# dmar-bonn/ipp-marl

Measured on AMD Instinct MI355X. Metric: agent-env steps/s (4 UAVs, 256x256 grid, random policy, env-step HIP kernels), higher is better.
Workload: dtype f32

## Files before the change

ipp-marl_amd/csrc/terrain.hip:

```cpp
#include "ippm_internal.h"

#define IPPM_DOMAIN_TERRAIN 3u

static inline hipStream_t S_(void* s) { return reinterpret_cast<hipStream_t>(s); }

__global__ __launch_bounds__(256) void k_terrain_noise(const ippm_config* __restrict__ c, const int64_t* __restrict__ episode,
                                                       float* __restrict__ noise, size_t cells) {
  const int e = blockIdx.y;
  const uint64_t ep = (uint64_t)episode[e];
  const uint32_t k0 = (uint32_t)c->philox_seed, k1 = (uint32_t)(c->philox_seed >> 32);
  const uint32_t sw = ippm_stream_word(0u, 0u, IPPM_DOMAIN_TERRAIN);
  float* out = noise + (size_t)e * cells;
  const size_t groups = (cells + 3) >> 2;
  for (size_t g = (size_t)blockIdx.x * blockDim.x + threadIdx.x; g < groups; g += (size_t)gridDim.x * blockDim.x) {
    Philox4 ph = ippm_philox((uint32_t)g, (uint32_t)ep, sw, (uint32_t)(ep >> 32), k0, k1);
    float z[4];
#pragma unroll
    for (int h = 0; h < 2; ++h) {
      const float u1 = ((float)(ph.v[2 * h] >> 8) + 1.0f) * (1.0f / 16777216.0f);
      const float u2 = (float)(ph.v[2 * h + 1] >> 8) * (1.0f / 16777216.0f);
      const float r = sqrtf(-2.0f * logf(u1));
      float s, co;
      sincospif(2.0f * u2, &s, &co);
      z[2 * h] = r * co;
      z[2 * h + 1] = r * s;
    }
    const size_t base = g << 2;
    if (base + 3 < cells && (cells & 3) == 0) {
      *reinterpret_cast<float4*>(out + base) = make_float4(z[0], z[1], z[2], z[3]);
    } else {
      for (int q = 0; q < 4 && base + q < cells; ++q) out[base + q] = z[q];
    }
  }
}


__device__ __forceinline__ float2 cmul(float2 a, float2 b) {
#pragma clang fp contract(off)
  const float p = a.y * b.y, q = a.y * b.x;
  return make_float2(__builtin_fmaf(a.x, b.x, -p), __builtin_fmaf(a.x, b.y, q));
}
__device__ __forceinline__ uint32_t bitrev(uint32_t v, int bits) { return __brev(v) >> (32 - bits); }

__device__ __forceinline__ uint32_t terrain_call(int gx, int gy, int cx, int ky) {
  return (uint32_t)(cx & (gx / 2 - 1)) * (uint32_t)(gy / 2 + 1) + (uint32_t)ky;
}
__device__ __forceinline__ float2 terrain_bin_from(uint32_t w1, uint32_t w2, bool self, bool conj, float amp) {
  const float u1 = ((float)(w1 >> 8) + 1.0f) * (1.0f / 16777216.0f);
  const float u2 = (float)(w2 >> 8) * (1.0f / 16777216.0f);
  const float r = __builtin_sqrtf(-1.3862943611f * __builtin_amdgcn_logf(u1));
  const float sn = __builtin_amdgcn_sinf(u2), cs = __builtin_amdgcn_cosf(u2);
  if (self) return make_float2(amp * 1.41421356237f * r * cs, 0.0f);
  return make_float2(amp * r * cs, conj ? -amp * r * sn : amp * r * sn);
}
__device__ __forceinline__ float2 terrain_bin(uint64_t ep, uint32_t k0, uint32_t k1, int gx, int gy, int kx, int ky, float amp) {
  const bool edge = ky == 0 || 2 * ky == gy;
  int cx = kx;
  bool conj = false;
  if (edge && 2 * kx > gx) { cx = gx - kx; conj = true; }
  const bool self = edge && (cx == 0 || 2 * cx == gx);
  Philox4 ph = ippm_philox(terrain_call(gx, gy, cx, ky), (uint32_t)ep, ippm_stream_word(0u, 1u, IPPM_DOMAIN_TERRAIN), (uint32_t)(ep >> 32), k0, k1);
  const bool upper = 2 * cx >= gx;
  return terrain_bin_from(upper ? ph.v[2] : ph.v[0], upper ? ph.v[3] : ph.v[1], self, conj, amp);
}
__device__ __forceinline__ void terrain_bin_pair(uint64_t ep, uint32_t k0, uint32_t k1, int gx, int gy, int kx, int ky, float amp_lo,
                                                 float amp_hi, float2& lo, float2& hi) {
  Philox4 ph = ippm_philox(terrain_call(gx, gy, kx, ky), (uint32_t)ep, ippm_stream_word(0u, 1u, IPPM_DOMAIN_TERRAIN), (uint32_t)(ep >> 32), k0, k1);
  lo = terrain_bin_from(ph.v[0], ph.v[1], false, false, amp_lo);
  hi = terrain_bin_from(ph.v[2], ph.v[3], false, false, amp_hi);
}

__global__ __launch_bounds__(256) void k_terrain_spectrum(const ippm_config* __restrict__ c, const int64_t* __restrict__ episode,
                                                          const float* __restrict__ amp, float2* __restrict__ spec) {
  const int e = blockIdx.y, gx = c->grid_x, gy = c->grid_y, hy = gy / 2 + 1;
  const uint64_t ep = (uint64_t)episode[e];
  const uint32_t k0 = (uint32_t)c->philox_seed, k1 = (uint32_t)(c->philox_seed >> 32);
  for (int i = blockIdx.x * blockDim.x + threadIdx.x; i < gx * hy; i += gridDim.x * blockDim.x)
    spec[(size_t)e * gx * hy + i] = terrain_bin(ep, k0, k1, gx, gy, i / hy, i % hy, amp[i]);
}

__device__ constexpr float TWC[16] = {1.000000000f, 0.980785280f, 0.923879533f, 0.831469612f, 0.707106781f, 0.555570233f,
                                      0.382683432f, 0.195090322f, 0.000000000f, -0.195090322f, -0.382683432f, -0.555570233f,
                                      -0.707106781f, -0.831469612f, -0.923879533f, -0.980785280f};
__device__ constexpr float TWS[16] = {0.000000000f, 0.195090322f, 0.382683432f, 0.555570233f, 0.707106781f, 0.831469612f,
                                      0.923879533f, 0.980785280f, 1.000000000f, 0.980785280f, 0.923879533f, 0.831469612f,
                                      0.707106781f, 0.555570233f, 0.382683432f, 0.195090322f};

template <int R>
__device__ __forceinline__ void fft_reg(float2 (&a)[R]) {
  constexpr int LOG = R == 8 ? 3 : (R == 16 ? 4 : 5);
  static_assert((1 << LOG) == R, "fft_reg: R must be 8, 16 or 32");
#pragma unroll
  for (int i = 0; i < R; ++i) {
    int j = 0;
#pragma unroll
    for (int b = 0; b < LOG; ++b) j |= ((i >> b) & 1) << (LOG - 1 - b);
    if (i < j) {
      const float2 t = a[i];
      a[i] = a[j];
      a[j] = t;
    }
  }
#pragma unroll
  for (int s = 0; s < LOG; ++s) {
#pragma unroll
    for (int j = 0; j < R / 2; ++j) {
      const int half = 1 << s, pos = j & (half - 1), i0 = ((j >> s) << (s + 1)) + pos, i1 = i0 + half, t = pos * (16 >> s);
      const float2 u = a[i0], v = cmul(a[i1], make_float2(TWC[t], TWS[t]));
      a[i0] = make_float2(u.x + v.x, u.y + v.y);
      a[i1] = make_float2(u.x - v.x, u.y - v.y);
    }
  }
}

template <int N1, int N2, int Q>
struct FourStep {
  static constexpr int SEQ = N1 * (N2 + 1) + 1;
  static constexpr int THREADS = Q * (N1 > N2 ? N1 : N2);
  float2 xbuf[Q * SEQ];
  float2 twn[N1 * N2];

  __device__ __forceinline__ void init_twiddles(const float2* __restrict__ roots1024) {
    for (int i = threadIdx.x; i < N1 * N2; i += THREADS) twn[i] = roots1024[i * (1024 / (N1 * N2))];
    __syncthreads();
  }
  __device__ __forceinline__ void run(float2 (&v)[N1], float2 (&o)[N2], int q_in, int i2, bool in_active, int q_out, int k1,
                                      bool out_active) {
    if (in_active) {
      fft_reg<N1>(v);
#pragma unroll
      for (int k = 0; k < N1; ++k) xbuf[q_in * SEQ + k * (N2 + 1) + i2] = cmul(v[k], twn[i2 * k]);
    }
    __syncthreads();
    if (out_active) {
#pragma unroll
      for (int i = 0; i < N2; ++i) o[i] = xbuf[q_out * SEQ + k1 * (N2 + 1) + i];
      fft_reg<N2>(o);
    }
  }
};

__device__ __forceinline__ uint32_t order_key(float f) {
  const uint32_t b = __float_as_uint(f);
  return (b & 0x80000000u) ? ~b : (b | 0x80000000u);
}
__device__ __forceinline__ float key_value(uint32_t k) { return __uint_as_float((k & 0x80000000u) ? (k & 0x7FFFFFFFu) : ~k); }

template <int N1, int N2, int Q, bool GEN>
__global__ __launch_bounds__((FourStep<N1, N2, Q>::THREADS)) void k_terrain_fft_x(const ippm_config* __restrict__ c,
                                                                               const int64_t* __restrict__ episode,
                                                                               const float* __restrict__ amp,
                                                                               const float2* __restrict__ spec,
                                                                               float2* __restrict__ work,
                                                                               uint32_t* __restrict__ range_keys,
                                                                               const float2* __restrict__ roots1024, int key_stride) {
  __shared__ FourStep<N1, N2, Q> fs;
  const int e = blockIdx.y, gx = N1 * N2, gy = c->grid_y, hy = gy / 2 + 1, tid = threadIdx.x;
  const bool edge_wg = blockIdx.x == gridDim.x - 1;
  if (range_keys && blockIdx.x == 0 && tid == 0) {
    range_keys[key_stride * e] = 0xFFFFFFFFu;
    range_keys[key_stride * e + 1] = 0u;
    if (key_stride == 4) {
      range_keys[4 * e + 2] = 0u;
      range_keys[4 * e + 3] = 0u;
      if (e == 0) range_keys[4 * gridDim.y] = 0u;
    }
  }
  fs.init_twiddles(roots1024);
  const int q_in = tid % Q, i2 = tid / Q, k1 = tid % N1, q_out = tid / N1;
  const bool in_active = i2 < N2, out_active = q_out < Q;
  auto column = [&](int q) { return edge_wg ? (q == 0 ? 0 : (q == 1 ? gy / 2 : -1)) : (1 + (int)blockIdx.x * Q + q < gy / 2 ? 1 + (int)blockIdx.x * Q + q : -1); };
  float2 v[N1], o[N2];
  if (in_active) {
    const int ky = column(q_in);
    const uint64_t ep = GEN ? (uint64_t)episode[e] : 0;
    const uint32_t k0 = (uint32_t)c->philox_seed, k1s = (uint32_t)(c->philox_seed >> 32);
#pragma unroll
    for (int i1 = 0; i1 < N1; ++i1) v[i1] = make_float2(0.0f, 0.0f);
    if (ky >= 0) {
      if (GEN && edge_wg) {
#pragma unroll
        for (int i1 = 0; i1 < N1; ++i1) {
          const int kx = i1 * N2 + i2;
          v[i1] = terrain_bin(ep, k0, k1s, gx, gy, kx, ky, amp[(size_t)kx * hy + ky]);
        }
      } else if (GEN) {
#pragma unroll
        for (int i1 = 0; i1 < N1 / 2; ++i1) {
          const int kx = i1 * N2 + i2;
          terrain_bin_pair(ep, k0, k1s, gx, gy, kx, ky, amp[(size_t)kx * hy + ky], amp[(size_t)(kx + gx / 2) * hy + ky], v[i1], v[i1 + N1 / 2]);
        }
      } else {
#pragma unroll
        for (int i1 = 0; i1 < N1; ++i1) v[i1] = spec[((size_t)e * gx + i1 * N2 + i2) * hy + ky];
      }
    }
  }
  fs.run(v, o, q_in, i2, in_active, q_out, k1, out_active);
  const int ky_out = out_active ? column(q_out) : -1;
  if (ky_out >= 0) {
    float2* dst = work + ((size_t)e * hy + ky_out) * gx + k1;
#pragma unroll
    for (int k2 = 0; k2 < N2; ++k2) dst[N1 * k2] = o[k2];
  }
}

template <int N1, int N2, int Q, int MODE>
__global__ __launch_bounds__((FourStep<N1, N2, Q>::THREADS)) void k_terrain_fft_y(const ippm_config* __restrict__ c,
                                                                               const float2* __restrict__ work,
                                                                               float* __restrict__ field,
                                                                               uint32_t* __restrict__ range_keys,
                                                                               const float2* __restrict__ roots1024,
                                                                               uint32_t* __restrict__ truth32, int truth_words, int key_stride) {
  __shared__ FourStep<N1, N2, Q> fs;
  const int tid = threadIdx.x, gx = c->grid_x, gy = N1 * N2, hy = gy / 2 + 1;
  int e = blockIdx.y, part = blockIdx.x;
  __shared__ uint32_t s_ticket, s_keys[2];
  if (MODE == 3) {
    if (tid == 0) s_ticket = atomicAdd(range_keys + 4 * gridDim.y, 1u);
  }
  fs.init_twiddles(roots1024);
  if (MODE == 3) {
    const uint32_t tk = s_ticket;
    e = (int)(tk / gridDim.x);
    part = (int)(tk - (uint32_t)e * gridDim.x);
  }
  const int x0 = part * 2 * Q;
  const int q_in = tid % Q, i2 = tid / Q, k1 = tid % N1, q_out = tid / N1;
  const bool in_active = i2 < N2, out_active = q_out < Q;
  float2 v[N1], o[N2];
  if (in_active) {
    const float2* src = work + (size_t)e * hy * gx + x0 + 2 * q_in;
#pragma unroll
    for (int i1 = 0; i1 < N1; ++i1) {
      const int i = i1 * N2 + i2, m = 2 * i > gy ? gy - i : i;
      const float4 ab = *reinterpret_cast<const float4*>(src + (size_t)m * gx);
      float2 a = make_float2(ab.x, ab.y), b = make_float2(ab.z, ab.w);
      if (2 * i > gy) { a.y = -a.y; b.y = -b.y; }
      if (i == 0 || 2 * i == gy) { a.y = 0.0f; b.y = 0.0f; }
      v[i1] = make_float2(a.x - b.y, a.y + b.x);
    }
  }
  fs.run(v, o, q_in, i2, in_active, q_out, k1, out_active);
  if (MODE != 2) {
    float lo = INFINITY, hi = -INFINITY;
    if (out_active) {
      float* dst = field + ((size_t)e * gx + x0 + 2 * q_out) * gy + k1;
#pragma unroll
      for (int k2 = 0; k2 < N2; ++k2) {
        if (MODE == 0) {
          dst[N1 * k2] = o[k2].x;
          dst[(size_t)gy + N1 * k2] = o[k2].y;
        }
        lo = fminf(lo, fminf(o[k2].x, o[k2].y));
        hi = fmaxf(hi, fmaxf(o[k2].x, o[k2].y));
      }
    }
    if (range_keys) {
#pragma unroll
      for (int m = 32; m > 0; m >>= 1) {
        lo = fminf(lo, __shfl_xor(lo, m, 64));
        hi = fmaxf(hi, __shfl_xor(hi, m, 64));
      }
      __shared__ float s_lo[8], s_hi[8];
      constexpr int NW = FourStep<N1, N2, Q>::THREADS / 64;
      if ((tid & 63) == 0) { s_lo[tid >> 6] = lo; s_hi[tid >> 6] = hi; }
      __syncthreads();
      if (tid == 0) {
        for (int w = 1; w < NW; ++w) { lo = fminf(lo, s_lo[w]); hi = fmaxf(hi, s_hi[w]); }
        if (MODE != 3) {
          atomicMin(range_keys + key_stride * e, order_key(lo));
          atomicMax(range_keys + key_stride * e + 1, order_key(hi));
        } else {
          uint32_t* rec = range_keys + 4 * e;
          const uint32_t o1 = __hip_atomic_fetch_min(rec, order_key(lo), __ATOMIC_RELAXED, __HIP_MEMORY_SCOPE_AGENT);
          const uint32_t o2 = __hip_atomic_fetch_max(rec + 1, order_key(hi), __ATOMIC_RELAXED, __HIP_MEMORY_SCOPE_AGENT);
          asm volatile("s_waitcnt vmcnt(0)" : : "v"(o1), "v"(o2) : "memory");
          __hip_atomic_fetch_add(rec + 2, 1u, __ATOMIC_RELAXED, __HIP_MEMORY_SCOPE_AGENT);
          unsigned spins = 0;
          while (atomicCAS(rec + 2, 0xFFFFFFFFu, 0xFFFFFFFEu) < gridDim.x) {
            __builtin_amdgcn_s_sleep(64);
            if (++spins > (1u << 21)) {
              atomicExch(rec + 3, 0xDEAD0000u | (unsigned)part);
              break;
            }
          }
          s_keys[0] = atomicCAS(rec, 0xFFFFFFFFu, 0xFFFFFFFEu);
          s_keys[1] = atomicCAS(rec + 1, 0xFFFFFFFFu, 0xFFFFFFFEu);
        }
      }
    }
    if (MODE != 3) return;
    __syncthreads();
  }
  {
    static_assert(N1 == 8 || N1 == 16 || N1 == 32, "a chunk must not straddle a 32-bit word");
    const uint32_t key_lo = MODE == 3 ? s_keys[0] : range_keys[key_stride * e];
    const uint32_t key_hi = MODE == 3 ? s_keys[1] : range_keys[key_stride * e + 1];
    const float lo = key_value(key_lo), span = key_value(key_hi) - lo;
    const int lane = tid & 63, rows_per_wave = 64 / N1;
    const int my_q = (tid >> 6) * rows_per_wave + lane;
    const bool storer = lane < rows_per_wave && my_q < Q;
    uint32_t* out = truth32 + (size_t)e * truth_words;
    const size_t row_a = ((size_t)(x0 + 2 * my_q) * gy) >> 5, row_b = ((size_t)(x0 + 2 * my_q + 1) * gy) >> 5;
    uint32_t wa = 0, wb = 0;
#pragma unroll
    for (int k2 = 0; k2 < N2; ++k2) {
      const uint64_t ba = __ballot(out_active && (o[k2].x - lo) / span >= 0.5f);
      const uint64_t bb = __ballot(out_active && (o[k2].y - lo) / span >= 0.5f);
      const uint32_t mask = N1 == 32 ? 0xFFFFFFFFu : ((1u << (N1 & 31)) - 1u);
      const int sh = (k2 * N1) & 31;
      wa |= ((uint32_t)(ba >> ((N1 * lane) & 63)) & mask) << sh;
      wb |= ((uint32_t)(bb >> ((N1 * lane) & 63)) & mask) << sh;
      if (((k2 + 1) * N1) % 32 == 0) {
        if (storer) { out[row_a + ((k2 * N1) >> 5)] = wa; out[row_b + ((k2 * N1) >> 5)] = wb; }
        wa = 0; wb = 0;
      }
    }
  }
}

#define IPPM_PACK_PARTS 4
__global__ __launch_bounds__(1024) void k_terrain_pack(const float* __restrict__ field, uint8_t* __restrict__ truth, size_t cells,
                                                       size_t truth_bytes) {
  __shared__ float s_lo[16], s_hi[16];
  const int e = blockIdx.y, tid = threadIdx.x, lane = tid & 63, wave = tid >> 6, nwave = blockDim.x >> 6;
  const float* f = field + (size_t)e * cells;
  float lo = INFINITY, hi = -INFINITY;
  if ((cells & 3) == 0) {
    const float4* f4 = reinterpret_cast<const float4*>(f);
    const size_t n4 = cells >> 2;
#pragma unroll 4
    for (size_t i = tid; i < n4; i += blockDim.x) {
      const float4 v = f4[i];
      lo = fminf(fminf(lo, fminf(v.x, v.y)), fminf(v.z, v.w));
      hi = fmaxf(fmaxf(hi, fmaxf(v.x, v.y)), fmaxf(v.z, v.w));
    }
  } else {
    for (size_t i = tid; i < cells; i += blockDim.x) {
      const float v = f[i];
      lo = fminf(lo, v);
      hi = fmaxf(hi, v);
    }
  }
#pragma unroll
  for (int o = 32; o > 0; o >>= 1) {
    lo = fminf(lo, __shfl_xor(lo, o, 64));
    hi = fmaxf(hi, __shfl_xor(hi, o, 64));
  }
  if (lane == 0) { s_lo[wave] = lo; s_hi[wave] = hi; }
  __syncthreads();
  lo = s_lo[0];
  hi = s_hi[0];
  for (int w = 1; w < nwave; ++w) {
    lo = fminf(lo, s_lo[w]);
    hi = fmaxf(hi, s_hi[w]);
  }
  const float span = hi - lo;
  uint32_t* out = reinterpret_cast<uint32_t*>(truth + (size_t)e * truth_bytes);
  const size_t words = truth_bytes >> 2;
  const size_t chunks = (cells + 63) >> 6;
  for (size_t ch = (size_t)blockIdx.x * nwave + wave; ch < chunks; ch += (size_t)gridDim.x * nwave) {
    const size_t i = (ch << 6) + lane;
    const bool one = i < cells && (f[i] - lo) / span >= 0.5f;
    const uint64_t bits = __ballot(one);
    if (lane < 2 && 2 * ch + lane < words) out[2 * ch + lane] = (uint32_t)(bits >> (32 * lane));
  }
}

__global__ __launch_bounds__(256) void k_terrain_pack_keys(const float* __restrict__ field, const uint32_t* __restrict__ range_keys,
                                                           uint8_t* __restrict__ truth, size_t cells, size_t truth_bytes) {
  const int e = blockIdx.y, lane = threadIdx.x & 63, wave = threadIdx.x >> 6, nwave = blockDim.x >> 6;
  const float* f = field + (size_t)e * cells;
  const float lo = key_value(range_keys[2 * e]), span = key_value(range_keys[2 * e + 1]) - lo;
  uint32_t* out = reinterpret_cast<uint32_t*>(truth + (size_t)e * truth_bytes);
  const size_t words = truth_bytes >> 2, chunks = (cells + 63) >> 6;
  const size_t stride = (size_t)gridDim.x * nwave;
  for (size_t ch0 = (size_t)blockIdx.x * nwave + wave; ch0 < chunks; ch0 += 4 * stride) {
    float v[4];
#pragma unroll
    for (int u = 0; u < 4; ++u) {
      const size_t i = ((ch0 + u * stride) << 6) + lane;
      v[u] = i < cells ? f[i] : lo;
    }
#pragma unroll
    for (int u = 0; u < 4; ++u) {
      const size_t ch = ch0 + u * stride;
      const uint64_t bits = __ballot(((ch << 6) + lane) < cells && (v[u] - lo) / span >= 0.5f);
      if (ch < chunks && lane < 2 && 2 * ch + lane < words) out[2 * ch + lane] = (uint32_t)(bits >> (32 * lane));
    }
  }
}

typedef float terrain_f4 __attribute__((ext_vector_type(4)));
__global__ __launch_bounds__(256) void k_terrain_pack_keys4(const float* __restrict__ field, const uint32_t* __restrict__ range_keys,
                                                            uint8_t* __restrict__ truth, size_t cells, size_t truth_bytes) {
  const int e = blockIdx.y;
  const size_t g = (size_t)blockIdx.x * 256 + threadIdx.x;
  const float lo = key_value(range_keys[2 * e]), span = key_value(range_keys[2 * e + 1]) - lo;
  uint32_t nib = 0;
  if (4 * g < cells) {
    const terrain_f4 v = __builtin_nontemporal_load(reinterpret_cast<const terrain_f4*>(field + (size_t)e * cells) + g);
    nib = ((v.x - lo) / span >= 0.5f ? 1u : 0u) | ((v.y - lo) / span >= 0.5f ? 2u : 0u) | ((v.z - lo) / span >= 0.5f ? 4u : 0u) |
          ((v.w - lo) / span >= 0.5f ? 8u : 0u);
  }
  uint32_t w = nib << (4 * (threadIdx.x & 7));
  w |= __shfl_xor(w, 1, 64);
  w |= __shfl_xor(w, 2, 64);
  w |= __shfl_xor(w, 4, 64);
  const size_t word = g >> 3;
  if ((threadIdx.x & 7) == 0 && word < (truth_bytes >> 2)) reinterpret_cast<uint32_t*>(truth + (size_t)e * truth_bytes)[word] = w;
}

extern "C" int ippm_terrain_noise(ippm_ctx* ctx, const int64_t* episode, float* noise, int32_t n_envs, void* stream) {
  if (!ctx || !episode || !noise) { ippm_set_error("ippm_terrain_noise: null argument"); return -1; }
  if (n_envs <= 0) return 0;
  const size_t cells = (size_t)ctx->cfg.grid_x * ctx->cfg.grid_y;
  const int gx = (int)std::min<size_t>(64, (cells / 4 + 255) / 256);
  hipLaunchKernelGGL(k_terrain_noise, dim3(gx > 0 ? gx : 1, n_envs), dim3(256), 0, S_(stream), ctx->dcfg, episode, noise, cells);
  IPPM_LAUNCH_CHECK("terrain_noise");
  return 0;
}

extern "C" int ippm_terrain_pack(ippm_ctx* ctx, const float* field, const uint32_t* range_keys, uint8_t* truth, int32_t n_envs,
                                 void* stream) {
  if (!ctx || !field || !truth) { ippm_set_error("ippm_terrain_pack: null argument"); return -1; }
  if (n_envs <= 0) return 0;
  const size_t cells = (size_t)ctx->cfg.grid_x * ctx->cfg.grid_y;
  if (range_keys && cells % 4 == 0 && (reinterpret_cast<uintptr_t>(field) & 15) == 0) {
    IPPM_LAUNCH(ctx, IPPM_T_TERRAIN, k_terrain_pack_keys4, dim3((unsigned)((cells / 4 + 255) / 256), n_envs), dim3(256), S_(stream), field,
                       range_keys, truth, cells, ippm_truth_bytes(ctx->cfg.grid_x, ctx->cfg.grid_y));
    IPPM_LAUNCH_CHECK("terrain_pack_keys4");
    return 0;
  }
  if (range_keys) {
    const int gxb = (int)std::min<size_t>(64, ((cells + 63) / 64 + 15) / 16);
    hipLaunchKernelGGL(k_terrain_pack_keys, dim3(gxb > 0 ? gxb : 1, n_envs), dim3(256), 0, S_(stream), field, range_keys, truth, cells,
                       ippm_truth_bytes(ctx->cfg.grid_x, ctx->cfg.grid_y));
    IPPM_LAUNCH_CHECK("terrain_pack_keys");
    return 0;
  }
  hipLaunchKernelGGL(k_terrain_pack, dim3(IPPM_PACK_PARTS, n_envs), dim3(1024), 0, S_(stream), field, truth, cells,
                     ippm_truth_bytes(ctx->cfg.grid_x, ctx->cfg.grid_y));
  IPPM_LAUNCH_CHECK("terrain_pack");
  return 0;
}

static bool terrain_side_ok(int n) { return n == 128 || n == 256 || n == 512 || n == 1024; }

static int terrain_pow2_check(const ippm_ctx* ctx, const char* who) {
  if (!terrain_side_ok(ctx->cfg.grid_x) || !terrain_side_ok(ctx->cfg.grid_y)) {
    ippm_set_error(std::string(who) + ": grid sides must be 128, 256, 512 or 1024 (use ippm_terrain_noise + an FFT library otherwise)");
    return -1;
  }
  return 0;
}

#define TERRAIN_DISPATCH(n, CALL)                \
  switch (n) {                                   \
    case 128: { CALL(8, 16, 16); break; }        \
    case 256: { CALL(16, 16, 16); break; }       \
    case 512: { CALL(16, 32, 8); break; }        \
    default: { CALL(32, 32, 4); break; }         \
  }

extern "C" int ippm_terrain_spectrum(ippm_ctx* ctx, const int64_t* episode, const float* amp, float* spec, int32_t n_envs,
                                     void* stream) {
  if (!ctx || !episode || !amp || !spec) { ippm_set_error("ippm_terrain_spectrum: null argument"); return -1; }
  if (terrain_pow2_check(ctx, "ippm_terrain_spectrum")) return -1;
  if (n_envs <= 0) return 0;
  const int bins = ctx->cfg.grid_x * (ctx->cfg.grid_y / 2 + 1);
  hipLaunchKernelGGL(k_terrain_spectrum, dim3(std::min(64, (bins + 255) / 256), n_envs), dim3(256), 0, S_(stream), ctx->dcfg,
                     episode, amp, reinterpret_cast<float2*>(spec));
  IPPM_LAUNCH_CHECK("terrain_spectrum");
  return 0;
}

static int terrain_launch_x(ippm_ctx* ctx, const int64_t* episode, const float* amp, const float2* spec2, float2* work2,
                            uint32_t* range_keys, int n_envs, hipStream_t st, int key_stride = 2) {
  const int gx = ctx->cfg.grid_x, gy = ctx->cfg.grid_y;
#define LAUNCH_X(N1, N2, Q)                                                                                                  \
  {                                                                                                                          \
    const dim3 grid((gy / 2 - 1 + Q - 1) / Q + 1, n_envs), block(FourStep<N1, N2, Q>::THREADS);                              \
    if (spec2) IPPM_LAUNCH(ctx, IPPM_T_TERRAIN, (k_terrain_fft_x<N1, N2, Q, false>), grid, block, st, ctx->dcfg, episode, amp, spec2, work2, \
                           range_keys, ctx->d_roots, key_stride);                                                            \
    else IPPM_LAUNCH(ctx, IPPM_T_TERRAIN, (k_terrain_fft_x<N1, N2, Q, true>), grid, block, st, ctx->dcfg, episode, amp, spec2, work2,        \
                     range_keys, ctx->d_roots, key_stride);                                                                  \
  }
  TERRAIN_DISPATCH(gx, LAUNCH_X)
#undef LAUNCH_X
  IPPM_LAUNCH_CHECK("terrain_fft_x");
  return 0;
}

template <int MODE>
static int terrain_launch_y(ippm_ctx* ctx, const float2* work2, float* field, uint32_t* range_keys, uint8_t* truth, int n_envs,
                            hipStream_t st, int key_stride = 2) {
  const int gx = ctx->cfg.grid_x, gy = ctx->cfg.grid_y;
#define LAUNCH_Y(N1, N2, Q)                                                                                                  \
  IPPM_LAUNCH(ctx, IPPM_T_TERRAIN, (k_terrain_fft_y<N1, N2, Q, MODE>), dim3(gx / (2 * Q), n_envs), dim3(FourStep<N1, N2, Q>::THREADS), st, \
              ctx->dcfg, work2, field, range_keys, ctx->d_roots, reinterpret_cast<uint32_t*>(truth), (int)(ippm_truth_bytes(gx, gy) >> 2),       \
              MODE == 3 ? 4 : key_stride)
  TERRAIN_DISPATCH(gy, LAUNCH_Y)
#undef LAUNCH_Y
  IPPM_LAUNCH_CHECK("terrain_fft_y");
  return 0;
}

extern "C" int ippm_terrain_field(ippm_ctx* ctx, const int64_t* episode, const float* amp, const float* spec, float* work,
                                  float* field, uint32_t* range_keys, int32_t n_envs, void* stream) {
  if (!ctx || !work || !field) { ippm_set_error("ippm_terrain_field: null argument"); return -1; }
  if (!spec && (!episode || !amp)) { ippm_set_error("ippm_terrain_field: needs either spec or (episode, amp)"); return -1; }
  if (terrain_pow2_check(ctx, "ippm_terrain_field")) return -1;
  if (n_envs <= 0) return 0;
  if (int rc = terrain_launch_x(ctx, episode, amp, reinterpret_cast<const float2*>(spec), reinterpret_cast<float2*>(work), range_keys, n_envs,
                                S_(stream))) return rc;
  return terrain_launch_y<0>(ctx, reinterpret_cast<const float2*>(work), field, range_keys, nullptr, n_envs, S_(stream));
}

extern "C" int ippm_terrain_truth(ippm_ctx* ctx, const int64_t* episode, const float* amp, float* work, uint32_t* range_keys,
                                  uint8_t* truth, int32_t n_envs, void* stream) {
  if (!ctx || !episode || !amp || !work || !range_keys || !truth) { ippm_set_error("ippm_terrain_truth: null argument"); return -1; }
  if (terrain_pow2_check(ctx, "ippm_terrain_truth")) return -1;
  if (n_envs <= 0) return 0;
  if (int rc = terrain_launch_x(ctx, episode, amp, nullptr, reinterpret_cast<float2*>(work), range_keys, n_envs, S_(stream), 4)) return rc;
  if (ctx->knob_terrain_one_launch && ctx->cfg.grid_x <= 512)
    return terrain_launch_y<3>(ctx, reinterpret_cast<const float2*>(work), nullptr, range_keys, truth, n_envs, S_(stream), 4);
  if (int rc = terrain_launch_y<1>(ctx, reinterpret_cast<const float2*>(work), nullptr, range_keys, nullptr, n_envs, S_(stream), 4)) return rc;
  return terrain_launch_y<2>(ctx, reinterpret_cast<const float2*>(work), nullptr, range_keys, truth, n_envs, S_(stream), 4);
}
```

Baseline: 29.32 million.

## Fuse terrain 2D FFT and threshold pack into one per-env on-chip kernel

Adds a single-block-per-environment kernel that runs the x-direction FFT, transposes through shared memory, runs the y-direction FFT, reduces min/max in-block, and writes the packed truth bits. For square grids up to 256 it is used when the one-launch knob is off, replacing the global work buffer round trip, the atomic range keys and the separate launches. In exchange each environment runs in one workgroup with large register arrays, so parallelism is limited to n_envs blocks and register pressure may spill. Shared helpers are factored out of the existing kernels.

```diff
diff --git a/ipp-marl_amd/csrc/terrain.hip b/ipp-marl_amd/csrc/terrain.hip
--- a/ipp-marl_amd/csrc/terrain.hip
+++ b/ipp-marl_amd/csrc/terrain.hip
@@ -145,6 +145,65 @@
   return (b & 0x80000000u) ? ~b : (b | 0x80000000u);
 }
 __device__ __forceinline__ float key_value(uint32_t k) { return __uint_as_float((k & 0x80000000u) ? (k & 0x7FFFFFFFu) : ~k); }
+
+
+template <int N1, int N2>
+__device__ __forceinline__ void terrain_draw_column(float2 (&v)[N1], uint64_t ep, uint32_t k0, uint32_t k1s, const float* __restrict__ amp,
+                                                    int gy, int i2, int ky, bool edge) {
+  constexpr int gx = N1 * N2;
+  const int hy = gy / 2 + 1;
+  if (edge) {
+#pragma unroll
+    for (int i1 = 0; i1 < N1; ++i1) {
+      const int kx = i1 * N2 + i2;
+      v[i1] = terrain_bin(ep, k0, k1s, gx, gy, kx, ky, amp[(size_t)kx * hy + ky]);
+    }
+  } else {
+#pragma unroll
+    for (int i1 = 0; i1 < N1 / 2; ++i1) {
+      const int kx = i1 * N2 + i2;
+      terrain_bin_pair(ep, k0, k1s, gx, gy, kx, ky, amp[(size_t)kx * hy + ky], amp[(size_t)(kx + gx / 2) * hy + ky], v[i1], v[i1 + N1 / 2]);
+    }
+  }
+}
+
+template <int N1, int N2>
+__device__ __forceinline__ void terrain_row_pair(float2 (&v)[N1], const float2* src, size_t stride, int i2) {
+  constexpr int gy = N1 * N2;
+#pragma unroll
+  for (int i1 = 0; i1 < N1; ++i1) {
+    const int i = i1 * N2 + i2, m = 2 * i > gy ? gy - i : i;
+    const float4 ab = *reinterpret_cast<const float4*>(src + (size_t)m * stride);
+    float2 a = make_float2(ab.x, ab.y), b = make_float2(ab.z, ab.w);
+    if (2 * i > gy) { a.y = -a.y; b.y = -b.y; }
+    if (i == 0 || 2 * i == gy) { a.y = 0.0f; b.y = 0.0f; }
+    v[i1] = make_float2(a.x - b.y, a.y + b.x);
+  }
+}
+
+template <int N1, int N2, int Q>
+__device__ __forceinline__ void terrain_threshold_pack(const float2 (&o)[N2], bool out_active, int t, float lo, float span,
+                                                       uint32_t* __restrict__ out, int x0, int gy) {
+  static_assert(N1 == 8 || N1 == 16 || N1 == 32, "a chunk must not straddle a 32-bit word");
+  const int lane = t & 63, rows_per_wave = 64 / N1;
+  const int my_q = (t >> 6) * rows_per_wave + lane;
+  const bool storer = lane < rows_per_wave && my_q < Q;
+  const size_t row_a = ((size_t)(x0 + 2 * my_q) * gy) >> 5, row_b = ((size_t)(x0 + 2 * my_q + 1) * gy) >> 5;
+  uint32_t wa = 0, wb = 0;
+#pragma unroll
+  for (int k2 = 0; k2 < N2; ++k2) {
+    const uint64_t ba = __ballot(out_active && (o[k2].x - lo) / span >= 0.5f);
+    const uint64_t bb = __ballot(out_active && (o[k2].y - lo) / span >= 0.5f);
+    const uint32_t mask = N1 == 32 ? 0xFFFFFFFFu : ((1u << (N1 & 31)) - 1u);
+    const int sh = (k2 * N1) & 31;
+    wa |= ((uint32_t)(ba >> ((N1 * lane) & 63)) & mask) << sh;
+    wb |= ((uint32_t)(bb >> ((N1 * lane) & 63)) & mask) << sh;
+    if (((k2 + 1) * N1) % 32 == 0) {
+      if (storer) { out[row_a + ((k2 * N1) >> 5)] = wa; out[row_b + ((k2 * N1) >> 5)] = wb; }
+      wa = 0; wb = 0;
+    }
+  }
+}
 
 template <int N1, int N2, int Q, bool GEN>
 __global__ __launch_bounds__((FourStep<N1, N2, Q>::THREADS)) void k_terrain_fft_x(const ippm_config* __restrict__ c,
@@ -178,18 +237,8 @@
 #pragma unroll
     for (int i1 = 0; i1 < N1; ++i1) v[i1] = make_float2(0.0f, 0.0f);
     if (ky >= 0) {
-      if (GEN && edge_wg) {
-#pragma unroll
-        for (int i1 = 0; i1 < N1; ++i1) {
-          const int kx = i1 * N2 + i2;
-          v[i1] = terrain_bin(ep, k0, k1s, gx, gy, kx, ky, amp[(size_t)kx * hy + ky]);
-        }
-      } else if (GEN) {
-#pragma unroll
-        for (int i1 = 0; i1 < N1 / 2; ++i1) {
-          const int kx = i1 * N2 + i2;
-          terrain_bin_pair(ep, k0, k1s, gx, gy, kx, ky, amp[(size_t)kx * hy + ky], amp[(size_t)(kx + gx / 2) * hy + ky], v[i1], v[i1 + N1 / 2]);
-        }
+      if (GEN) {
+        terrain_draw_column<N1, N2>(v, ep, k0, k1s, amp, gy, i2, ky, edge_wg);
       } else {
 #pragma unroll
         for (int i1 = 0; i1 < N1; ++i1) v[i1] = spec[((size_t)e * gx + i1 * N2 + i2) * hy + ky];
@@ -230,16 +279,7 @@
   const bool in_active = i2 < N2, out_active = q_out < Q;
   float2 v[N1], o[N2];
   if (in_active) {
-    const float2* src = work + (size_t)e * hy * gx + x0 + 2 * q_in;
-#pragma unroll
-    for (int i1 = 0; i1 < N1; ++i1) {
-      const int i = i1 * N2 + i2, m = 2 * i > gy ? gy - i : i;
-      const float4 ab = *reinterpret_cast<const float4*>(src + (size_t)m * gx);
-      float2 a = make_float2(ab.x, ab.y), b = make_float2(ab.z, ab.w);
-      if (2 * i > gy) { a.y = -a.y; b.y = -b.y; }
-      if (i == 0 || 2 * i == gy) { a.y = 0.0f; b.y = 0.0f; }
-      v[i1] = make_float2(a.x - b.y, a.y + b.x);
-    }
+    terrain_row_pair<N1, N2>(v, work + (size_t)e * hy * gx + x0 + 2 * q_in, (size_t)gx, i2);
   }
   fs.run(v, o, q_in, i2, in_active, q_out, k1, out_active);
   if (MODE != 2) {
@@ -294,30 +334,108 @@
     __syncthreads();
   }
   {
-    static_assert(N1 == 8 || N1 == 16 || N1 == 32, "a chunk must not straddle a 32-bit word");
     const uint32_t key_lo = MODE == 3 ? s_keys[0] : range_keys[key_stride * e];
     const uint32_t key_hi = MODE == 3 ? s_keys[1] : range_keys[key_stride * e + 1];
     const float lo = key_value(key_lo), span = key_value(key_hi) - lo;
-    const int lane = tid & 63, rows_per_wave = 64 / N1;
-    const int my_q = (tid >> 6) * rows_per_wave + lane;
-    const bool storer = lane < rows_per_wave && my_q < Q;
-    uint32_t* out = truth32 + (size_t)e * truth_words;
-    const size_t row_a = ((size_t)(x0 + 2 * my_q) * gy) >> 5, row_b = ((size_t)(x0 + 2 * my_q + 1) * gy) >> 5;
-    uint32_t wa = 0, wb = 0;
-#pragma unroll
-    for (int k2 = 0; k2 < N2; ++k2) {
-      const uint64_t ba = __ballot(out_active && (o[k2].x - lo) / span >= 0.5f);
-      const uint64_t bb = __ballot(out_active && (o[k2].y - lo) / span >= 0.5f);
-      const uint32_t mask = N1 == 32 ? 0xFFFFFFFFu : ((1u << (N1 & 31)) - 1u);
-      const int sh = (k2 * N1) & 31;
-      wa |= ((uint32_t)(ba >> ((N1 * lane) & 63)) & mask) << sh;
-      wb |= ((uint32_t)(bb >> ((N1 * lane) & 63)) & mask) << sh;
-      if (((k2 + 1) * N1) % 32 == 0) {
-        if (storer) { out[row_a + ((k2 * N1) >> 5)] = wa; out[row_b + ((k2 * N1) >> 5)] = wb; }
-        wa = 0; wb = 0;
+    terrain_threshold_pack<N1, N2, Q>(o, out_active, tid, lo, span, truth32 + (size_t)e * truth_words, x0, gy);
+  }
+}
+
+template <int N1, int N2, int Q>
+struct TerrainOnChip {
+  using FS = FourStep<N1, N2, Q>;
+  static constexpr int N = N1 * N2, HY = N / 2 + 1, SUB = FS::THREADS, THREADS = 2 * SUB;
+  static constexpr int NB = (N / 2 - 1 + Q - 1) / Q + 1, NBS = (NB + 1) / 2;
+  static constexpr int NYB = N / (2 * Q), NYS = NYB / 2;
+  static constexpr int K2PB = 2 * Q / N1;
+  static constexpr int SROW = 2 * Q + 2;
+  static_assert(SUB % 64 == 0 && NYB % 2 == 0 && K2PB * N1 == 2 * Q && NYB * K2PB == N2, "TerrainOnChip: geometry");
+  FS fs[2];
+  alignas(16) float2 slice[2][HY * SROW];
+  float s_lo[THREADS / 64], s_hi[THREADS / 64];
+};
+
+template <int N1, int N2, int Q>
+__global__ __launch_bounds__((TerrainOnChip<N1, N2, Q>::THREADS)) void k_terrain_onchip(const ippm_config* __restrict__ c,
+                                                                                     const int64_t* __restrict__ episode,
+                                                                                     const float* __restrict__ amp,
+                                                                                     const float2* __restrict__ roots1024,
+                                                                                     uint32_t* __restrict__ truth32, int truth_words) {
+  using G = TerrainOnChip<N1, N2, Q>;
+  __shared__ alignas(16) G s;
+  constexpr int n = G::N;
+  const int e = blockIdx.x, tid = threadIdx.x;
+  const int sg = __builtin_amdgcn_readfirstlane(tid / G::SUB), t = tid % G::SUB;
+  typename G::FS& fs = s.fs[sg];
+  for (int i = t; i < n; i += G::SUB) fs.twn[i] = roots1024[i * (1024 / n)];
+  __syncthreads();
+  const int q_in = t % Q, i2 = t / Q, k1 = t % N1, q_out = t / N1;
+  const bool in_active = i2 < N2, out_active = q_out < Q;
+  auto column = [&](int b, int q) {
+    if (b >= G::NB) return -1;
+    if (b == G::NB - 1) return q == 0 ? 0 : (q == 1 ? n / 2 : -1);
+    return 1 + b * Q + q < n / 2 ? 1 + b * Q + q : -1;
+  };
+  const uint64_t ep = (uint64_t)episode[e];
+  const uint32_t k0 = (uint32_t)c->philox_seed, k1s = (uint32_t)(c->philox_seed >> 32);
+
+  float2 T[G::NBS][N2];
+#pragma unroll
+  for (int j = 0; j < G::NBS; ++j) {
+    const int b = 2 * j + sg;
+    const bool edge = 2 * j + 1 >= G::NB - 1 && b == G::NB - 1;
+    float2 v[N1];
+#pragma unroll
+    for (int i1 = 0; i1 < N1; ++i1) v[i1] = make_float2(0.0f, 0.0f);
+#pragma unroll
+    for (int k2 = 0; k2 < N2; ++k2) T[j][k2] = make_float2(0.0f, 0.0f);
+    const int ky = in_active ? column(b, q_in) : -1;
+    if (ky >= 0) terrain_draw_column<N1, N2>(v, ep, k0, k1s, amp, n, i2, ky, edge);
+    if (j > 0) __syncthreads();
+    fs.run(v, T[j], q_in, i2, in_active && b < G::NB, q_out, k1, out_active && b < G::NB);
+  }
+
+  float2 R[G::NYS][N2];
+  float lo = INFINITY, hi = -INFINITY;
+#pragma unroll
+  for (int jy = 0; jy < G::NYS; ++jy) {
+    if (out_active) {
+#pragma unroll
+      for (int j = 0; j < G::NBS; ++j) {
+        const int ky = column(2 * j + sg, q_out);
+        if (ky >= 0) {
+#pragma unroll
+          for (int h = 0; h < 2; ++h)
+#pragma unroll
+            for (int kk = 0; kk < G::K2PB; ++kk) s.slice[h][ky * G::SROW + k1 + N1 * kk] = T[j][(2 * jy + h) * G::K2PB + kk];
+        }
       }
     }
-  }
+    __syncthreads();
+    float2 v[N1];
+    if (in_active) terrain_row_pair<N1, N2>(v, &s.slice[sg][2 * q_in], (size_t)G::SROW, i2);
+    fs.run(v, R[jy], q_in, i2, in_active, q_out, k1, out_active);
+    if (out_active) {
+#pragma unroll
+      for (int k2 = 0; k2 < N2; ++k2) {
+        lo = fminf(lo, fminf(R[jy][k2].x, R[jy][k2].y));
+        hi = fmaxf(hi, fmaxf(R[jy][k2].x, R[jy][k2].y));
+      }
+    }
+  }
+#pragma unroll
+  for (int m = 32; m > 0; m >>= 1) {
+    lo = fminf(lo, __shfl_xor(lo, m, 64));
+    hi = fmaxf(hi, __shfl_xor(hi, m, 64));
+  }
+  if ((tid & 63) == 0) { s.s_lo[tid >> 6] = lo; s.s_hi[tid >> 6] = hi; }
+  __syncthreads();
+#pragma unroll
+  for (int w = 0; w < G::THREADS / 64; ++w) { lo = fminf(lo, s.s_lo[w]); hi = fmaxf(hi, s.s_hi[w]); }
+  const float span = hi - lo;
+#pragma unroll
+  for (int jy = 0; jy < G::NYS; ++jy)
+    terrain_threshold_pack<N1, N2, Q>(R[jy], out_active, t, lo, span, truth32 + (size_t)e * truth_words, (2 * jy + sg) * 2 * Q, n);
 }
 
 #define IPPM_PACK_PARTS 4
@@ -523,6 +641,16 @@
   if (!ctx || !episode || !amp || !work || !range_keys || !truth) { ippm_set_error("ippm_terrain_truth: null argument"); return -1; }
   if (terrain_pow2_check(ctx, "ippm_terrain_truth")) return -1;
   if (n_envs <= 0) return 0;
+  const int gx = ctx->cfg.grid_x, gy = ctx->cfg.grid_y;
+  if (!ctx->knob_terrain_one_launch && gx == gy && gx <= 256) {
+#define LAUNCH_ONCHIP(N1, N2, Q)                                                                                                      \
+  IPPM_LAUNCH(ctx, IPPM_T_TERRAIN, (k_terrain_onchip<N1, N2, Q>), dim3(n_envs), dim3(TerrainOnChip<N1, N2, Q>::THREADS), S_(stream), \
+              ctx->dcfg, episode, amp, ctx->d_roots, reinterpret_cast<uint32_t*>(truth), (int)(ippm_truth_bytes(gx, gy) >> 2))
+    if (gx == 128) LAUNCH_ONCHIP(8, 16, 16); else LAUNCH_ONCHIP(16, 16, 16);
+#undef LAUNCH_ONCHIP
+    IPPM_LAUNCH_CHECK("terrain_onchip");
+    return 0;
+  }
   if (int rc = terrain_launch_x(ctx, episode, amp, nullptr, reinterpret_cast<float2*>(work), range_keys, n_envs, S_(stream), 4)) return rc;
   if (ctx->knob_terrain_one_launch && ctx->cfg.grid_x <= 512)
     return terrain_launch_y<3>(ctx, reinterpret_cast<const float2*>(work), nullptr, range_keys, truth, n_envs, S_(stream), 4);
```

New measurement: 28.97 million. 1.2% lower.
